# OedonLestrange42/GNURadio-WiFI-ImageTransfer

Measured on NVIDIA B200. Metric: rx_msamples_per_s, higher is better.
Workload: dtype f32+u8

## Files before the change

### gnuradio-wifi-imagetransfer_b200/csrc/rx_kernels.cuh

```cuda
#pragma once
#include <cuda_pipeline.h>
#include "viterbi.cuh"

__device__ __forceinline__ cf fe_at(const cf *x, int64_t j, int hist) { return j < -(int64_t)hist ? cf{0.f, 0.f} : x[j]; }

__device__ __forceinline__ int find_link(const LinkDesc *links, int n_links, int64_t chunk)
{
    int lo = 0, hi = n_links - 1;
    while (lo < hi) {
        int mid = (lo + hi + 1) >> 1;
        if (links[mid].chunk_base <= chunk) lo = mid; else hi = mid - 1;
    }
    return lo;
}

#ifndef DET_BLOCK
#define DET_BLOCK 32
#endif
#define DET_SPLIT (DET_THREADS / DET_BLOCK)
#define DET_ROWS (DET_BLOCK + 2)
#define DET_STRIDE 66
#define DET_SMEM_BYTES (DET_ROWS * DET_STRIDE * (int)sizeof(cf) + 32)

__device__ __forceinline__ uint32_t det_smem_u32(const void *p) { return (uint32_t)__cvta_generic_to_shared(p); }
// ... 472 lines not shown
        if ((tid & 31) == 0) { rmax[tid >> 5] = bm; ridx[tid >> 5] = bi; }
        __syncthreads();
        if (tid == 0) {
            for (int w = 1; w < SL_THREADS / 32; ++w)
                if (rmax[w] > bm || (rmax[w] == bm && ridx[w] < bi)) { bm = rmax[w]; bi = ridx[w]; }
            top[r] = bi;
            smag[bi] = -2.f;
        }
        __syncthreads();
    }
    if (tid == 0) {
        int found = 0, fs = SYNC_LENGTH;
        float fo = 0.f;
        for (int i = 0; i < 3 && found != 64; ++i)
            for (int k = i + 1; k < 4; ++k) {
                int lo = min(top[i], top[k]), hi = max(top[i], top[k]);
                int diff = hi - lo;
                if (diff == 63 || diff == 64 || diff == 65) {
                    cf first = scorr[lo], second = scorr[hi];
                    cf pr = wdm_cmulc(first, second);
                    fs = lo;
                    fo = wdm_atan2f(pr.im, pr.re) / (float)diff;
                    found = diff;
                    if (diff == 64) break;
                }
            }
        frames[f].found = found;
        frames[f].frame_start = fs;
        frames[f].freq_long = fo;
    }
}

#ifndef DEMOD_MINB
#define DEMOD_MINB 5
#endif
struct DemodParams {
    double bw, freq;
    int algo;
    int want_carrier;
    int soft;
};

__device__ __forceinline__ int emitted_symbols(int avail, int fs, bool last)
{
    int R = avail - fs;
    if (R <= 0) return 0;
    int E = R <= 128 ? R : 128 + 64 * ((R - 128) / 80) + max(0, ((R - 128) % 80) - 16);
    return last ? E / 64 : (E + 63) / 64;
}

template <bool SOFT, int ALGO, int PHASE>
__global__ void __launch_bounds__(128, DEMOD_MINB) k_demod(const cf *__restrict__ iq, const LinkDesc *__restrict__ links, wifi_b200_frame *frames, int f0, int n_frames,
                                                EqState *states, uint8_t *rows, cf *carrier, DemodParams prm,
                                                const uint16_t *__restrict__ depunct_lut, uint32_t *__restrict__ vit_in,
                                                int8_t *__restrict__ soft_rows, uint32_t *__restrict__ vit_soft_in)
{
    __shared__ int8_t s_soft[SOFT ? 4 : 1][SOFT ? 392 : 4];
    __shared__ uint16_t s_slut[SOFT ? 4 : 1][SOFT ? 432 : 2];
    __shared__ float s_h2[SOFT ? 4 : 1][SOFT ? 64 : 2];
    __shared__ cf s_hu[4][64];
    __shared__ double s_md[4][64], s_ms[4][64];
    __shared__ uint16_t s_lut[4][432];
    __shared__ __align__(8) uint8_t s_bits[4][49 * 8];
    constexpr int phase = PHASE;
    const int wib = threadIdx.x >> 5, lane = threadIdx.x & 31;
    const int f = f0 + blockIdx.x * 4 + wib;
    if (f >= n_frames) return;
    const wifi_b200_frame F = frames[f];
    if (phase == 1 && F.burst_len < SYNC_LENGTH + 63) return;
    const LinkDesc L = links[F.link];
    const cf *x = iq + L.x_off;
    const bool last = L.is_final && (f == L.frame_first + L.frame_count - 1);
    float fo = F.freq_long;
    if (phase == 0) {
        if (!F.found) {
            fo = L.fo_carry;
            for (int g = f - 1; g >= L.frame_first; --g)
                if (frames[g].found) { fo = frames[g].freq_long; break; }
        }
        if (F.burst_len < SYNC_LENGTH + 63) {
            if (lane == 0 && F.n_syms >= 0) frames[f].freq_long = fo;
            return;
        }
    }
    const int avail = F.burst_len - SYNC_LENGTH;
    const int fs = F.frame_start;
    const int n_syms = emitted_symbols(avail, fs, last);
    const float fshort = F.freq_short;
    const float delta = fo - fshort;
    const cf w1 = crot(delta);
    const int64_t t = F.trigger;
    const int hist = L.hist;

    const int iA = lane + 32, iB = lane;
    const bool usedA = (iA <= 58), usedB = (iB >= 6);
    const bool dcA = (iA == 32);
    const int carA = c_tab.carrier_of[iA], carB = c_tab.carrier_of[iB];
    const float ltsA = c_tab.lts[iA], ltsB = c_tab.lts[iB];
    const int q0 = 2 * dev_bitrev5(lane);
    const WarpTw tw = warp_tw(lane, false);

    cf HA = {0.f, 0.f}, HB = {0.f, 0.f};
    cf pp[4] = {{0.f, 0.f}, {0.f, 0.f}, {0.f, 0.f}, {0.f, 0.f}};
    double d_er = 0.0, eps0, snr = 0.0;
    float havg = 1.f, w0A = 1.f, w0B = 1.f;
    int frame_symbols = 0, enc = 0, nb = 1;
    int n_begin, n_end;
    EqState *st = states + f;
    if (phase == 0) {
        eps0 = ((double)fshort - (double)fo) * prm.bw / (2 * M_PI * prm.freq);
        n_begin = 0;
        n_end = n_syms < 3 ? n_syms : 3;
        if (lane == 0) { frames[f].freq_long = fo; frames[f].n_syms = n_syms; }
    } else {
        if (!F.sig_ok) return;
        frame_symbols = F.frame_symbols;
        enc = F.encoding;
        nb = c_tab.mcs[enc].n_bpsc;
        HA = st->H[iA]; HB = st->H[iB];
#pragma unroll
        for (int q = 0; q < 4; ++q) pp[q] = st->prev_pil[q];
        d_er = st->d_er; eps0 = st->eps0;
        if (SOFT) { havg = st->havg; w0A = st->w0[iA]; w0B = st->w0[iB]; }
        n_begin = 3;
        n_end = n_syms < frame_symbols + 3 ? n_syms : frame_symbols + 3;
    }
    const int ndbps = c_tab.mcs[enc].n_dbps;
    const int wps = (phase == 1 && (ndbps & 7) == 0 && frame_symbols <= WIFI_MAX_SYM && F.length <= WIFI_MAX_PSDU) ? ndbps >> 3 : 0;
    uint32_t era_word = 0;
    if (wps) {
        for (int i = lane; i < 2 * ndbps; i += 32) {
            uint16_t e = depunct_lut[enc * 432 + i];
            s_lut[wib][(i & 15) * 27 + (i >> 4)] = (e == 0xffffu) ? (uint16_t)(48 << 3) : e;
        }
        if (lane < wps)
            for (int k = 0; k < 16; ++k)
                if (depunct_lut[enc * 432 + 16 * lane + k] == 0xffffu) era_word |= 2u << (2 * k);
        if (lane == 0) *reinterpret_cast<uint2 *>(&s_bits[wib][48 * 8]) = make_uint2(0u, 0u);
        __syncwarp();
    }
    uint32_t *vw = vit_in + (int64_t)f * VIT_MAXW;
    const bool soft_on = SOFT && phase == 1;
    const int swps = (soft_on && frame_symbols <= WIFI_MAX_SYM && F.length <= WIFI_MAX_PSDU) ? ndbps >> 1 : 0;
    if (SOFT && soft_on) {
        for (int i = lane; i < 2 * ndbps; i += 32) {
            uint16_t e = depunct_lut[enc * 432 + i];
            s_slut[wib][i] = (e == 0xffffu) ? 384 : e;
        }
        if (lane == 0) s_soft[wib][384] = 0;
        __syncwarp();
    }
    uint32_t *vsw = vit_soft_in ? vit_soft_in + (int64_t)f * SOFT_MAXW : nullptr;
    int n_rows = 0;
    auto sym_j0 = [&](int n) { return fs + ((n < 2) ? 64 * n + q0 : 128 + 80 * (n - 2) + 16 + q0); };
    auto fetch_raw = [&](int n, cf (&raw)[2]) {
        const int j0 = sym_j0(n);
#pragma unroll
        for (int u = 0; u < 2; ++u) {
            const int j = j0 + u;
            const int64_t src = t + j - 16;
            raw[u] = (j < avail && src >= -(int64_t)hist) ? x[src] : cf{0.f, 0.f};
        }
    };
    cf raw[2] = {{0.f, 0.f}, {0.f, 0.f}};
    if (n_begin < n_end) fetch_raw(n_begin, raw);
    int pidx = n_begin >= 2 ? (n_begin - 2) % 127 : 0;
    for (int n = n_begin; n < n_end; ++n) {
        if (PHASE == 1) __builtin_assume(n >= 3);
        cf a, b;
        {
            const int j0 = sym_j0(n);
            const cf s0 = raw[0], s1 = raw[1];
            if (n + 1 < n_end) fetch_raw(n + 1, raw);
            const cf r0 = crot(delta * (float)j0);
            const cf r1 = cmul(r0, w1);
            a = (j0 < avail) ? cmul(s0, r0) : cf{0.f, 0.f};
            b = (j0 + 1 < avail) ? cmul(s1, r1) : cf{0.f, 0.f};
        }
        warp_fft64(a, b, lane, tw);
        {
            double k = 2 * M_PI * n * 80 * (eps0 + d_er);
            double phA = k * (iA - 32) / 64, phB = k * (iB - 32) / 64;
            a = cmul(a, crot((float)phA));
            b = cmul(b, crot((float)phB));
        }
        cf c11 = cshfl(b, 11), c25 = cshfl(b, 25), c39 = cshfl(a, 7), c53 = cshfl(a, 21);
        const float p = (n >= 2) ? c_tab.polarity[pidx] : 1.f;
        if (n >= 2) pidx = pidx == 126 ? 0 : pidx + 1;
        cf pil[4];
        double beta;
        cf sbeta;
        if (n < 2) {
            sbeta = cadd(cadd(csub(c11, c25), c39), c53);
            pil[0] = c11; pil[1] = cf{-c25.re, -c25.im}; pil[2] = c39; pil[3] = c53;
        } else {
            pil[0] = cscale(c11, p); pil[1] = cscale(c25, p); pil[2] = cscale(c39, p); pil[3] = cscale(c53, -p);
            sbeta = cadd(cadd(cadd(pil[0], pil[2]), pil[1]), pil[3]);
        }
        cf ser = {0.f, 0.f};
        if (n >= 2) {
#pragma unroll
            for (int q = 0; q < 4; ++q) ser = wdm_cmacc(ser, pil[q], pp[q]);
        }
        const bool up = lane >= 16;
        const float at = wdm_atan2f(up ? ser.im : sbeta.im, up ? ser.re : sbeta.re);
        beta = (double)__shfl_sync(0xffffffffu, at, 0);
        double er = 0.0;
        if (n >= 2) {
            er = (double)__shfl_sync(0xffffffffu, at, 16);
            er *= prm.bw / (2 * M_PI * prm.freq * 80);
        }
#pragma unroll
        for (int q = 0; q < 4; ++q) pp[q] = pil[q];
        const cf wb = crot((float)(-beta));
        a = cmul(a, wb);
        b = cmul(b, wb);
        if (n >= 2) d_er = (1 - 0.1) * d_er + 0.1 * er;

        if (ALGO == WIFI_EQ_COMB) {
            cf r11 = cmul(c11, wb), r25 = cmul(c25, wb), r39 = cmul(c39, wb), r53 = cmul(c53, wb);
            cf cp[4];
            if (n < 2) { cp[0] = r11; cp[1] = cf{-r25.re, -r25.im}; cp[2] = r39; cp[3] = r53; }
            else { cp[0] = cscale(r11, p); cp[1] = cscale(r25, p); cp[2] = cscale(r39, p); cp[3] = cscale(r53, -p); }
            cf avg = cscale(cadd(cadd(cadd(cp[0], cp[1]), cp[2]), cp[3]), 0.25f);
#pragma unroll
            for (int u = 0; u < 2; ++u) {
                int i = u ? iB : iA;
                cf G;
                if (i <= 11) G = cadd(cscale(avg, (float)(11 - i) / 11.0f), cscale(cp[0], (float)i / 11.0f));
                else if (i <= 25) G = cadd(cscale(cp[0], (float)(25 - i) / 14.0f), cscale(cp[1], (float)(i - 11) / 14.0f));
                else if (i <= 39) G = cadd(cscale(cp[1], (float)(39 - i) / 14.0f), cscale(cp[2], (float)(i - 25) / 14.0f));
                else if (i <= 53) G = cadd(cscale(cp[2], (float)(53 - i) / 14.0f), cscale(cp[3], (float)(i - 39) / 14.0f));
                else G = cadd(cscale(cp[3], (float)(64 - i) / 11.0f), cscale(avg, (float)(i - 53) / 11.0f));
                if (u) b = cdiv(b, G); else a = cdiv(a, G);
            }
        }
        if (n == 0) {
            HA = a; HB = b;
        } else if (n == 1) {
            {
                cf d = csub(HA, a), s = cadd(HA, a);
                float md = sqrtf(d.re * d.re + d.im * d.im), ms = sqrtf(s.re * s.re + s.im * s.im);
                s_md[wib][iA] = (double)md * (double)md; s_ms[wib][iA] = (double)ms * (double)ms;
                if (usedA && !dcA) HA = cdiv(s, cf{ltsA * 2.0f, 0.f});
                d = csub(HB, b); s = cadd(HB, b);
                md = sqrtf(d.re * d.re + d.im * d.im); ms = sqrtf(s.re * s.re + s.im * s.im);
                s_md[wib][iB] = (double)md * (double)md; s_ms[wib][iB] = (double)ms * (double)ms;
                if (usedB) HB = cdiv(s, cf{ltsB * 2.0f, 0.f});
            }
            if (SOFT) {
                s_h2[wib][iA] = HA.re * HA.re + HA.im * HA.im;
                s_h2[wib][iB] = HB.re * HB.re + HB.im * HB.im;
            }
            __syncwarp();
            if (lane == 0) {
                double signal = 0, noise = 0;
                float acc = 0.f;
                for (int i = 6; i <= 58; ++i) {
                    if (i == 32) continue;
                    noise += s_md[wib][i];
                    signal += s_ms[wib][i];
                    if (SOFT) acc += s_h2[wib][i];
                }
                snr = 10 * log10(signal / noise / 2);
                havg = acc / 52.0f;
            }
            if (SOFT) {
                havg = __shfl_sync(0xffffffffu, havg, 0);
                w0A = s_h2[wib][iA] / havg;
                w0B = s_h2[wib][iB] / havg;
            }
            __syncwarp();
        } else {
            cf symA = {0.f, 0.f}, symB = {0.f, 0.f};
            int bitsA = 0, bitsB = 0;
            cf huA = {0.f, 0.f}, huB = {0.f, 0.f};
            SoftQ sqA, sqB;
#pragma unroll
            for (int u = 0; u < 2; ++u)
#pragma unroll
                for (int t = 0; t < 3; ++t) { sqA.q[u][t] = 0; sqB.q[u][t] = 0; }
            if (carA >= 0) {
                cf ptA;
                symA = cdiv(a, HA);
                dev_decide_point(nb, symA, bitsA, ptA);
                if (SOFT && soft_on) sqA = dev_soft_demap(nb, symA, w0A);
                if (ALGO == WIFI_EQ_LMS) {
                    cf q = cdiv(a, ptA);
                    HA = cadd(cscale(HA, 0.5f), cscale(q, 0.5f));
                } else if (ALGO == WIFI_EQ_STA) huA = cdiv(a, ptA);
            } else if (iA == 39) huA = cscale(a, p);
            else if (iA == 53) huA = cscale(a, -p);
            if (carB >= 0) {
                cf ptB;
                symB = cdiv(b, HB);
                dev_decide_point(nb, symB, bitsB, ptB);
                if (SOFT && soft_on) sqB = dev_soft_demap(nb, symB, w0B);
                if (ALGO == WIFI_EQ_LMS) {
                    cf q = cdiv(b, ptB);
                    HB = cadd(cscale(HB, 0.5f), cscale(q, 0.5f));
                } else if (ALGO == WIFI_EQ_STA) huB = cdiv(b, ptB);
            } else if (iB == 11 || iB == 25) huB = cscale(b, p);
            if (ALGO == WIFI_EQ_STA) {
                s_hu[wib][iA] = huA; s_hu[wib][iB] = huB;
                __syncwarp();
#pragma unroll
                for (int u = 0; u < 2; ++u) {
                    int i = u ? iB : iA;
                    if (i < 6 || i > 58 || i == 32) continue;
                    cf sum = {0.f, 0.f};
                    int cnt = 0;
                    for (int k = i - 2; k <= i + 2; ++k) {
                        if (k == 32 || k < 6 || k > 58) continue;
                        sum = cadd(sum, s_hu[wib][k]);
                        ++cnt;
                    }
                    cf avg = {sum.re / (float)cnt, sum.im / (float)cnt};
                    if (u) HB = cadd(cscale(HB, 0.5f), cscale(avg, 0.5f));
                    else HA = cadd(cscale(HA, 0.5f), cscale(avg, 0.5f));
                }
                __syncwarp();
            }
            if (n == 2) {
                if (carA >= 0) st->sig_bits[carA] = (uint8_t)bitsA;
                if (carB >= 0) st->sig_bits[carB] = (uint8_t)bitsB;
            } else {
                int64_t row = F.row_off + (n - 3);
                if (carA >= 0) rows[row * 48 + carA] = (uint8_t)bitsA;
                if (carB >= 0) rows[row * 48 + carB] = (uint8_t)bitsB;
                if (prm.want_carrier) {
                    if (carA >= 0) carrier[row * 48 + carA] = symA;
                    if (carB >= 0) carrier[row * 48 + carB] = symB;
                }
                if (wps) {
                    if (carA >= 0)
                        *reinterpret_cast<uint2 *>(&s_bits[wib][carA * 8]) =
                            make_uint2((((uint32_t)bitsA & 15u) * 0x00204081u) & 0x01010101u, (((uint32_t)bitsA >> 4) * 0x81u) & 0x0101u);
                    if (carB >= 0)
                        *reinterpret_cast<uint2 *>(&s_bits[wib][carB * 8]) =
                            make_uint2((((uint32_t)bitsB & 15u) * 0x00204081u) & 0x01010101u, (((uint32_t)bitsB >> 4) * 0x81u) & 0x0101u);
                    __syncwarp();
                    if (lane < wps) {
                        uint32_t word = era_word;
#pragma unroll
                        for (int k = 0; k < 16; ++k) {
                            const uint32_t e = s_lut[wib][k * 27 + lane];
                            word += (uint32_t)s_bits[wib][e] << (2 * k);
                        }
                        vw[(n - 3) * wps + lane] = word;
                    }
                    __syncwarp();
                }
                if (SOFT && soft_on) {
                    const int hb = nb > 1 ? nb >> 1 : 1;
#pragma unroll
                    for (int u = 0; u < 2; ++u)
#pragma unroll
                        for (int t = 0; t < 3; ++t) {
                            if (t < hb && (u == 0 || nb > 1)) {
                                const int k = u * hb + t;
                                if (carA >= 0) { s_soft[wib][(carA << 3) | k] = (int8_t)sqA.q[u][t]; soft_rows[row * SOFT_ROW + carA * nb + k] = (int8_t)sqA.q[u][t]; }
                                if (carB >= 0) { s_soft[wib][(carB << 3) | k] = (int8_t)sqB.q[u][t]; soft_rows[row * SOFT_ROW + carB * nb + k] = (int8_t)sqB.q[u][t]; }
                            }
                        }
                    __syncwarp();
                    for (int w = lane; w < swps; w += 32) {
                        uint32_t word = 0;
#pragma unroll
                        for (int k = 0; k < 4; ++k) word |= (uint32_t)(uint8_t)s_soft[wib][s_slut[wib][4 * w + k]] << (8 * k);
                        vsw[(n - 3) * swps + w] = word;
                    }
                    __syncwarp();
                }
                ++n_rows;
            }
        }
    }
    if (phase == 0) {
        st->H[iA] = HA; st->H[iB] = HB;
        if (SOFT) { st->w0[iA] = w0A; st->w0[iB] = w0B; }
        if (lane == 0) {
#pragma unroll
            for (int q = 0; q < 4; ++q) st->prev_pil[q] = pp[q];
            st->d_er = d_er; st->eps0 = eps0; st->snr = snr; st->havg = havg;
        }
    } else if (lane == 0) {
        frames[f].n_rows = n_rows;
    }
}

__global__ void __launch_bounds__(VIT_BLOCK) k_signal(wifi_b200_frame *frames, int f0, int n_frames, const EqState *states)
{
    __shared__ uint32_t ring[5 * 16 * VIT_BLOCK];
    __shared__ uint4 s_bm[8 * 4 * 16];
    const int tid = threadIdx.x;
    for (int i = tid; i < 512; i += VIT_BLOCK) s_bm[i] = VitCoreH::table_entry(i >> 6, (i >> 4) & 3, (uint32_t)(i & 15));
    __syncthreads();
    int f = f0 + blockIdx.x * VIT_BLOCK + tid;
    if (f >= n_frames) return;
    if (frames[f].n_syms < 3) return;
    const EqState *st = states + f;
    uint64_t lo = 0, hi = 0;
    for (int tstep = 0; tstep < 24; ++tstep) {
        int i0 = 2 * tstep, i1 = i0 + 1;
        uint32_t s0 = st->sig_bits[(i0 % 16) * 3 + i0 / 16] & 1u, s1 = st->sig_bits[(i1 % 16) * 3 + i1 / 16] & 1u;
        uint64_t nib = s0 | (s1 << 2);
        if (tstep < 16) lo |= nib << (4 * tstep); else hi |= nib << (4 * (tstep - 16));
    }
    VitCoreH v;
    v.init();
    const uint32_t first = (uint32_t)lo;
    v.step4<0>(s_bm, 0xau, 0xau, first & 0xfu, (first >> 4) & 0xfu);
    v.step4<4>(s_bm, (first >> 8) & 0xfu, (first >> 12) & 0xfu, (first >> 16) & 0xfu, (first >> 20) & 0xfu);
    v.trace_begin(ring, 1, 5, tid, true, 0xfcu);
    uint32_t dec = 0;
#pragma unroll 1
    for (int chunk = 1; chunk < 8; ++chunk) {
        const uint32_t bits = (uint32_t)(lo >> 24);
        lo = (lo >> 32) | (hi << 32);
// ... 499 lines not shown
```

### gnuradio-wifi-imagetransfer_b200/csrc/wifi_b200.cu

```cuda
#include <sched.h>

#include <cfloat>
#include <cmath>
#include <cstdio>
#include <cstdlib>
#include <cstring>
#include <mutex>
#include <string>
#include <deque>
#include <vector>

#include "rx_kernels.cuh"
#include "tx_kernels.cuh"


namespace {

const McsDesc H_MCS[8] = {
    {1, 48, 24, 0x0D, 0}, {1, 48, 36, 0x0F, 2}, {2, 96, 48, 0x05, 0}, {2, 96, 72, 0x07, 2},
    {4, 192, 96, 0x09, 0}, {4, 192, 144, 0x0B, 2}, {6, 288, 192, 0x01, 1}, {6, 288, 216, 0x03, 2},
};
const int H_LTS53[53] = {1, 1, -1, -1, 1, 1, -1, 1, -1, 1, 1, 1, 1, 1, 1, -1, -1, 1, 1, -1, 1, -1, 1, 1, 1, 1, 0,
                         1, -1, -1, 1, 1, -1, 1, -1, 1, -1, -1, -1, -1, -1, 1, 1, -1, -1, 1, -1, 1, -1, 1, 1, 1, 1};

// ... 490 lines not shown
        }
        if (timed) mark(h, ST_DETECT);
        if (tiles_g > 0)
            k_detect<<<(unsigned)(DET_SPLIT * tiles_g), DET_BLOCK, DET_SMEM, s>>>(iq, gl, ng, tile_base, tile_base + tiles_g, thr_f, h->d_flags, h->d_summary);
        if (timed) mark(h, ST_SELECT);
        if (tiles_g > 0)
            k_select_spec<<<(unsigned)((tiles_g * 32 + 127) / 128), 128, 0, s>>>(h->d_flags, h->d_summary, gl, ng, tile_base, tile_base + tiles_g,
                                                                                h->cfg.min_plateau, h->d_spec_trig, h->d_spec_cnt);
        if (tiles_g > 0)
            k_select_fix<<<(unsigned)((tiles_g * 32 + 127) / 128), 128, 0, s>>>(h->d_flags, h->d_summary, gl, ng, tile_base, tile_base + tiles_g,
                                                                               h->cfg.min_plateau, h->d_spec_trig, h->d_spec_cnt, h->d_spec_trig2, h->d_spec_cnt2);
        k_select<<<(ng * 32 + 127) / 128, 128, 0, s>>>(h->d_flags, h->d_summary, gl, ng, h->cfg.min_plateau, h->d_trig_tmp, h->d_spec_trig, h->d_spec_cnt2,
                                                       h->d_spec_trig2);
        k_reserve<<<1, 1024, 0, s>>>(gl, ng, h->d_counters, (unsigned long long *)(h->d_counters + 8), h->cfg.max_frames, h->d_counters + 2,
                                     (long long)frame_base, (long long)row_base);
        k_frames_init<<<dim3(8, ng), 128, 0, s>>>(gl, h->d_trig_tmp, h->d_frames, lb);
        if (timed) mark(h, ST_SYNC_LONG);
        CK(cudaMemcpyAsync(h->h_counters, h->d_counters, 64, cudaMemcpyDeviceToHost, s));
        CK(cudaStreamSynchronize(s));
        if (h->h_counters[2] != 0 || h->h_counters[0] > h->cfg.max_frames) {
            h->err = "more sync_short triggers than max_frames";
            return WIFI_E_OVERFLOW;
        }
        const int64_t f_end = h->h_counters[0], nf = f_end - frame_base;
        const int64_t rows_needed = *(int64_t *)(h->h_counters + 8);
        if (rows_needed > h->row_cap) {
            h->err = "row capacity exceeded";
            return WIFI_E_OVERFLOW;
        }
        const int f0 = (int)frame_base, fe = (int)f_end;
        if (nf > 0) {
            k_sync_long<<<(unsigned)nf, SL_THREADS, 0, s>>>(iq, h->d_links, h->d_frames, f0, fe);
            if (timed) mark(h, ST_DEMOD_HEAD);
            demod_head<<<(unsigned)((nf + 3) / 4), 128, 0, s>>>(iq, h->d_links, h->d_frames, f0, fe, h->d_states, h->d_rows, h->d_carrier, prm,
                                                            h->d_depunct, h->d_vit_in, h->d_soft, h->d_vit_soft_in);
            if (timed) mark(h, ST_SIGNAL);
            k_signal<<<(unsigned)((nf + VIT_BLOCK - 1) / VIT_BLOCK), VIT_BLOCK, 0, s>>>(h->d_frames, f0, fe, h->d_states);
            if (timed) mark(h, ST_DEMOD_DATA);
            demod_data<<<(unsigned)((nf + 3) / 4), 128, 0, s>>>(iq, h->d_links, h->d_frames, f0, fe, h->d_states, h->d_rows, h->d_carrier, prm,
                                                            h->d_depunct, h->d_vit_in, h->d_soft, h->d_vit_soft_in);
            if (timed) mark(h, ST_PLAN);
            CK(cudaMemsetAsync(h->d_link_dirty + lb, 0, (size_t)ng * sizeof(int), s));
            CK(cudaMemsetAsync(h->d_link_dirty + MAX_LINKS + lb, 0xff, (size_t)ng * sizeof(int), s));
            CK(cudaMemsetAsync(h->d_counters + 1, 0, sizeof(int), s));
            k_plan_fast<<<(unsigned)((nf + 127) / 128), 128, 0, s>>>(h->d_frames, f0, fe, h->d_jobs, h->d_pack_list, h->d_counters + 1, h->d_link_dirty, soft);
            k_plan<<<(ng * 32 + 127) / 128, 128, 0, s>>>(gl, ng, h->d_frames, h->d_jobs, h->d_pack_list, h->d_counters + 1,
                                                         h->d_counters + 2, soft, h->d_link_dirty + lb, h->d_link_dirty + MAX_LINKS + lb);
            if (timed) mark(h, ST_PACK);
            if (!soft) {
                k_pack<<<dim3(7, 148), 256, 0, s>>>(h->d_jobs, h->d_pack_list, h->d_counters + 1, h->d_rows, h->d_depunct, h->d_vit_in, h->d_frames);
                if (timed) mark(h, ST_VITERBI);
                auto launch_viterbi = [&](cudaStream_t st, int a, int b) {
                    const int64_t n = b - a;
                    const int form = h->viterbi_form ? h->viterbi_form : (n <= VW_SWITCH ? 1 : (n <= VQ_SWITCH ? 2 : 3));
                    if (form == 1) k_viterbi_warp<<<(unsigned)((n + VW_WARPS - 1) / VW_WARPS), 32 * VW_WARPS, 0, st>>>(h->d_jobs, a, b, h->d_vit_in, h->d_psdu, h->d_frames);
                    else if (form == 2) k_viterbi_quad<<<(unsigned)((n + VQ_FRAMES - 1) / VQ_FRAMES), VQ_BLOCK, 0, st>>>(h->d_jobs, a, b, h->d_vit_in, h->d_psdu, h->d_frames);
                    else k_viterbi<<<(unsigned)((n + VIT_BLOCK - 1) / VIT_BLOCK), VIT_BLOCK, vit_smem, st>>>(h->d_jobs, a, b, h->d_vit_in, h->d_psdu, h->d_frames);
                };
                const int64_t wave = (int64_t)h->sm_count * 2 * VIT_BLOCK;
                int64_t rem = nf % wave;
                if (rem > VQ_SPLIT_MAX) rem = 0;
                if (h->viterbi_form || nf < wave || rem == 0) {
                    launch_viterbi(s, f0, fe);
                } else {
                    CK(cudaEventRecord(h->ev_fork, s));
                    CK(cudaStreamWaitEvent(h->aux_stream, h->ev_fork, 0));
                    launch_viterbi(h->aux_stream, fe - (int)rem, fe);
                    launch_viterbi(s, f0, fe - (int)rem);
                    CK(cudaEventRecord(h->ev_join, h->aux_stream));
                    CK(cudaStreamWaitEvent(s, h->ev_join, 0));
                }
            } else {
// ... 1125 lines not shown
```

### gnuradio-wifi-imagetransfer_b200/csrc/wifi_common.cuh

```cuda
#pragma once
#include <cuda_runtime.h>
#include <stdint.h>
#include "../../include/wifi_b200.h"
#include "../../include/wifi_detmath.h"

#define WIFI_MAX_SYM 511
#define WIFI_MAX_PSDU 1528
#define SS_MIN_GAP 480
#define SS_MAX_SAMPLES 43200
#define SYNC_LENGTH 320
#define FE_CHUNK 64
#define DET_THREADS 128
#define DET_TILE (DET_THREADS * FE_CHUNK)
#define PSDU_STRIDE 1536
#define VIT_MAXW 1560
#define SOFT_MAXW 6240
#define SOFT_ROW 288

typedef wdm_cf cf;
__device__ __forceinline__ cf cadd(cf a, cf b) { return {a.re + b.re, a.im + b.im}; }
__device__ __forceinline__ cf csub(cf a, cf b) { return {a.re - b.re, a.im - b.im}; }
__device__ __forceinline__ cf cmul(cf a, cf b) { return wdm_cmul(a, b); }
__device__ __forceinline__ cf cdiv(cf a, cf b) { return wdm_cdiv(a, b); }
__device__ __forceinline__ cf cscale(cf a, float s) { return {a.re * s, a.im * s}; }
// ... 131 lines not shown
#pragma unroll
    for (int s = 0; s < 5; ++s) {
        const int half = 1 << s;
        t.w[s] = c_tab.tw[(lane & (half - 1)) * (32 >> s)];
    }
    t.w[5] = c_tab.tw[lane];
    if (inverse) {
#pragma unroll
        for (int s = 0; s < 6; ++s) t.w[s].im = -t.w[s].im;
    }
    return t;
}

__device__ __forceinline__ void warp_fft64(cf &a, cf &b, int lane, const WarpTw &tw)
{
#pragma unroll
    for (int s = 0; s < 5; ++s) {
        const int half = 1 << s;
        const cf w = tw.w[s];
        const bool hi = (lane & half) != 0;
        cf ta = hi ? cmul(w, a) : a;
        cf tb = hi ? cmul(w, b) : b;
        cf ra = cshfl_xor(ta, half);
        cf rb = cshfl_xor(tb, half);
        a = hi ? csub(ra, ta) : cadd(a, ra);
        b = hi ? csub(rb, tb) : cadd(b, rb);
    }
    cf t = cmul(tw.w[5], b);
    cf u = a;
    a = cadd(u, t);
    b = csub(u, t);
}

__device__ __forceinline__ int dev_soft_q(float l, float w)
{
    float v = rintf((l * w) * 16.0f);
    if (v > 32.f) v = 32.f;
    if (v < -32.f) v = -32.f;
    if (!(v == v)) v = 0.f;
    return (int)v;
}
struct SoftQ { int q[2][3]; };
__device__ __forceinline__ SoftQ dev_soft_demap(int nb, cf s, float w)
{
    SoftQ r;
#pragma unroll
    for (int u = 0; u < 2; ++u)
#pragma unroll
        for (int t = 0; t < 3; ++t) r.q[u][t] = 0;
    if (nb == 1) { r.q[0][0] = dev_soft_q(s.re, w); return r; }
    const int h = nb >> 1;
    const float level = (h == 1) ? sqrtf(0.5f) : (h == 2) ? sqrtf(0.1f) : sqrtf(1.0f / 42.0f);
    const float ax[2] = {s.re / level, s.im / level};
#pragma unroll
    for (int u = 0; u < 2; ++u) {
        const float a = ax[u], m = fabsf(a);
        r.q[u][0] = dev_soft_q(a, w);
        if (h == 2) r.q[u][1] = dev_soft_q(2.0f - m, w);
        if (h == 3) {
            r.q[u][1] = dev_soft_q(4.0f - m, w);
            r.q[u][2] = dev_soft_q(2.0f - fabsf(m - 4.0f), w);
        }
    }
    return r;
}
```

Before: 46750.

## Process each frame with a half-warp in demod, eight frames per block

The demod kernel now maps one frame to 16 lanes instead of a full warp. Each lane holds four FFT bins and uses a new half-warp radix FFT (four shuffle stages plus two in-register stages). Depuncture words are built from a uint4-vectorised LUT, and launch bounds and the grid are retuned to eight frames per block. The aim is to cut shuffle count and idle lanes per frame and raise frame-level parallelism. The cost is more registers, predicated execution to keep half-warps in lockstep, and extra loop iterations when the two frames sharing a warp differ in symbol count.

After: 49500, median of 6. 5.9% higher.

```diff
diff --git a/gnuradio-wifi-imagetransfer_b200/csrc/rx_kernels.cuh b/gnuradio-wifi-imagetransfer_b200/csrc/rx_kernels.cuh
--- a/gnuradio-wifi-imagetransfer_b200/csrc/rx_kernels.cuh
+++ b/gnuradio-wifi-imagetransfer_b200/csrc/rx_kernels.cuh
@@ -528,8 +528,9 @@
 }
 
 #ifndef DEMOD_MINB
-#define DEMOD_MINB 5
+#define DEMOD_MINB 4
 #endif
+#define DEMOD_FPB 8
 struct DemodParams {
     double bw, freq;
     int algo;
@@ -546,37 +547,40 @@
 }
 
 template <bool SOFT, int ALGO, int PHASE>
-__global__ void __launch_bounds__(128, DEMOD_MINB) k_demod(const cf *__restrict__ iq, const LinkDesc *__restrict__ links, wifi_b200_frame *frames, int f0, int n_frames,
+__global__ void __launch_bounds__(32 * DEMOD_FPB / 2, DEMOD_MINB) k_demod(const cf *__restrict__ iq, const LinkDesc *__restrict__ links, wifi_b200_frame *frames, int f0, int n_frames,
                                                 EqState *states, uint8_t *rows, cf *carrier, DemodParams prm,
                                                 const uint16_t *__restrict__ depunct_lut, uint32_t *__restrict__ vit_in,
                                                 int8_t *__restrict__ soft_rows, uint32_t *__restrict__ vit_soft_in)
 {
-    __shared__ int8_t s_soft[SOFT ? 4 : 1][SOFT ? 392 : 4];
-    __shared__ uint16_t s_slut[SOFT ? 4 : 1][SOFT ? 432 : 2];
-    __shared__ float s_h2[SOFT ? 4 : 1][SOFT ? 64 : 2];
-    __shared__ cf s_hu[4][64];
-    __shared__ double s_md[4][64], s_ms[4][64];
-    __shared__ uint16_t s_lut[4][432];
-    __shared__ __align__(8) uint8_t s_bits[4][49 * 8];
+    constexpr int BITS = 49 * 8;
+    __shared__ int8_t s_soft[SOFT ? DEMOD_FPB * BITS : 4];
+    __shared__ uint16_t s_slut[SOFT ? DEMOD_FPB : 1][SOFT ? 432 : 2];
+    __shared__ float s_h2[SOFT ? DEMOD_FPB : 1][SOFT ? 64 : 2];
+    __shared__ cf s_hu[DEMOD_FPB][64];
+    __shared__ double s_md[DEMOD_FPB][64], s_ms[DEMOD_FPB][64];
+    __shared__ __align__(16) uint32_t s_lut[DEMOD_FPB][27 * 20];
+    __shared__ __align__(8) uint8_t s_bits[DEMOD_FPB * BITS];
     constexpr int phase = PHASE;
-    const int wib = threadIdx.x >> 5, lane = threadIdx.x & 31;
-    const int f = f0 + blockIdx.x * 4 + wib;
-    if (f >= n_frames) return;
-    const wifi_b200_frame F = frames[f];
-    if (phase == 1 && F.burst_len < SYNC_LENGTH + 63) return;
+    const int fib = threadIdx.x >> 4, l = threadIdx.x & 15;
+    const unsigned hmask = 0xffffu << (threadIdx.x & 16);
+    const int f = f0 + blockIdx.x * DEMOD_FPB + fib;
+    if (f0 + blockIdx.x * DEMOD_FPB + (fib & ~1) >= n_frames) return;
+    bool ok = f < n_frames;
+    const wifi_b200_frame F = frames[ok ? f : f - 1];
+    if (phase == 1 && F.burst_len < SYNC_LENGTH + 63) ok = false;
     const LinkDesc L = links[F.link];
     const cf *x = iq + L.x_off;
     const bool last = L.is_final && (f == L.frame_first + L.frame_count - 1);
     float fo = F.freq_long;
-    if (phase == 0) {
+    if (phase == 0 && ok) {
         if (!F.found) {
             fo = L.fo_carry;
             for (int g = f - 1; g >= L.frame_first; --g)
                 if (frames[g].found) { fo = frames[g].freq_long; break; }
         }
         if (F.burst_len < SYNC_LENGTH + 63) {
-            if (lane == 0 && F.n_syms >= 0) frames[f].freq_long = fo;
-            return;
+            if (l == 0 && F.n_syms >= 0) frames[f].freq_long = fo;
+            ok = false;
         }
     }
     const int avail = F.burst_len - SYNC_LENGTH;
@@ -588,99 +592,117 @@
     const int64_t t = F.trigger;
     const int hist = L.hist;
 
-    const int iA = lane + 32, iB = lane;
-    const bool usedA = (iA <= 58), usedB = (iB >= 6);
-    const bool dcA = (iA == 32);
-    const int carA = c_tab.carrier_of[iA], carB = c_tab.carrier_of[iB];
-    const float ltsA = c_tab.lts[iA], ltsB = c_tab.lts[iB];
-    const int q0 = 2 * dev_bitrev5(lane);
-    const WarpTw tw = warp_tw(lane, false);
-
-    cf HA = {0.f, 0.f}, HB = {0.f, 0.f};
+    int bin[4], car[4];
+#pragma unroll
+    for (int k = 0; k < 4; ++k) {
+        bin[k] = (l + 16 * k + 32) & 63;
+        car[k] = c_tab.carrier_of[bin[k]];
+    }
+    const int q0 = 4 * (int)(__brev((unsigned)l) >> 28);
+    const HalfTw tw = half_tw(l);
+
+    cf H[4] = {{0.f, 0.f}, {0.f, 0.f}, {0.f, 0.f}, {0.f, 0.f}};
+    float w0[4] = {1.f, 1.f, 1.f, 1.f};
     cf pp[4] = {{0.f, 0.f}, {0.f, 0.f}, {0.f, 0.f}, {0.f, 0.f}};
     double d_er = 0.0, eps0, snr = 0.0;
-    float havg = 1.f, w0A = 1.f, w0B = 1.f;
+    float havg = 1.f;
     int frame_symbols = 0, enc = 0, nb = 1;
     int n_begin, n_end;
     EqState *st = states + f;
     if (phase == 0) {
         eps0 = ((double)fshort - (double)fo) * prm.bw / (2 * M_PI * prm.freq);
         n_begin = 0;
-        n_end = n_syms < 3 ? n_syms : 3;
-        if (lane == 0) { frames[f].freq_long = fo; frames[f].n_syms = n_syms; }
+        n_end = !ok ? 0 : n_syms < 3 ? n_syms : 3;
+        if (ok && l == 0) { frames[f].freq_long = fo; frames[f].n_syms = n_syms; }
     } else {
-        if (!F.sig_ok) return;
+        ok = ok && F.sig_ok;
+        n_begin = n_end = 3;
+    }
+    if (phase == 1 && ok) {
         frame_symbols = F.frame_symbols;
         enc = F.encoding;
         nb = c_tab.mcs[enc].n_bpsc;
-        HA = st->H[iA]; HB = st->H[iB];
+#pragma unroll
+        for (int k = 0; k < 4; ++k) H[k] = st->H[bin[k]];
 #pragma unroll
         for (int q = 0; q < 4; ++q) pp[q] = st->prev_pil[q];
         d_er = st->d_er; eps0 = st->eps0;
-        if (SOFT) { havg = st->havg; w0A = st->w0[iA]; w0B = st->w0[iB]; }
-        n_begin = 3;
+        if (SOFT) {
+            havg = st->havg;
+#pragma unroll
+            for (int k = 0; k < 4; ++k) w0[k] = st->w0[bin[k]];
+        }
         n_end = n_syms < frame_symbols + 3 ? n_syms : frame_symbols + 3;
     }
     const int ndbps = c_tab.mcs[enc].n_dbps;
-    const int wps = (phase == 1 && (ndbps & 7) == 0 && frame_symbols <= WIFI_MAX_SYM && F.length <= WIFI_MAX_PSDU) ? ndbps >> 3 : 0;
-    uint32_t era_word = 0;
+    const int wps = (phase == 1 && ok && (ndbps & 7) == 0 && frame_symbols <= WIFI_MAX_SYM && F.length <= WIFI_MAX_PSDU) ? ndbps >> 3 : 0;
+    uint32_t era_word[2] = {0u, 0u};
     if (wps) {
-        for (int i = lane; i < 2 * ndbps; i += 32) {
-            uint16_t e = depunct_lut[enc * 432 + i];
-            s_lut[wib][(i & 15) * 27 + (i >> 4)] = (e == 0xffffu) ? (uint16_t)(48 << 3) : e;
-        }
-        if (lane < wps)
-            for (int k = 0; k < 16; ++k)
-                if (depunct_lut[enc * 432 + 16 * lane + k] == 0xffffu) era_word |= 2u << (2 * k);
-        if (lane == 0) *reinterpret_cast<uint2 *>(&s_bits[wib][48 * 8]) = make_uint2(0u, 0u);
-        __syncwarp();
+        for (int i = l; i < 2 * ndbps; i += 16) {
+            const uint16_t e = depunct_lut[enc * 432 + i];
+            s_lut[fib][(i >> 4) * 20 + (i & 15)] = fib * BITS + ((e == 0xffffu) ? 48 << 3 : e);
+        }
+#pragma unroll
+        for (int j = 0; j < 2; ++j) {
+            const int w = l + 16 * j;
+            if (w < wps)
+                for (int k = 0; k < 16; ++k)
+                    if (depunct_lut[enc * 432 + 16 * w + k] == 0xffffu) era_word[j] |= 2u << (2 * k);
+        }
+        if (l == 0) *reinterpret_cast<uint2 *>(&s_bits[fib * BITS + 48 * 8]) = make_uint2(0u, 0u);
+        __syncwarp(hmask);
     }
     uint32_t *vw = vit_in + (int64_t)f * VIT_MAXW;
     const bool soft_on = SOFT && phase == 1;
-    const int swps = (soft_on && frame_symbols <= WIFI_MAX_SYM && F.length <= WIFI_MAX_PSDU) ? ndbps >> 1 : 0;
-    if (SOFT && soft_on) {
-        for (int i = lane; i < 2 * ndbps; i += 32) {
-            uint16_t e = depunct_lut[enc * 432 + i];
-            s_slut[wib][i] = (e == 0xffffu) ? 384 : e;
-        }
-        if (lane == 0) s_soft[wib][384] = 0;
-        __syncwarp();
+    const int swps = (soft_on && ok && frame_symbols <= WIFI_MAX_SYM && F.length <= WIFI_MAX_PSDU) ? ndbps >> 1 : 0;
+    if (SOFT && swps) {
+        for (int i = l; i < 2 * ndbps; i += 16) {
+            const uint16_t e = depunct_lut[enc * 432 + i];
+            s_slut[fib][i] = (uint16_t)(fib * BITS + ((e == 0xffffu) ? 384 : e));
+        }
+        if (l == 0) s_soft[fib * BITS + 384] = 0;
+        __syncwarp(hmask);
     }
     uint32_t *vsw = vit_soft_in ? vit_soft_in + (int64_t)f * SOFT_MAXW : nullptr;
     int n_rows = 0;
     auto sym_j0 = [&](int n) { return fs + ((n < 2) ? 64 * n + q0 : 128 + 80 * (n - 2) + 16 + q0); };
-    auto fetch_raw = [&](int n, cf (&raw)[2]) {
+    auto fetch_raw = [&](int n, cf (&raw)[4]) {
         const int j0 = sym_j0(n);
 #pragma unroll
-        for (int u = 0; u < 2; ++u) {
+        for (int u = 0; u < 4; ++u) {
             const int j = j0 + u;
             const int64_t src = t + j - 16;
             raw[u] = (j < avail && src >= -(int64_t)hist) ? x[src] : cf{0.f, 0.f};
         }
     };
-    cf raw[2] = {{0.f, 0.f}, {0.f, 0.f}};
+    cf raw[4] = {{0.f, 0.f}, {0.f, 0.f}, {0.f, 0.f}, {0.f, 0.f}};
     if (n_begin < n_end) fetch_raw(n_begin, raw);
     int pidx = n_begin >= 2 ? (n_begin - 2) % 127 : 0;
-    for (int n = n_begin; n < n_end; ++n) {
+    const int n_stop = max(n_end, __shfl_xor_sync(0xffffffffu, n_end, 16));
+    for (int n = n_begin; n < n_stop; ++n) {
         if (PHASE == 1) __builtin_assume(n >= 3);
-        cf a, b;
+        const bool act = n < n_end;
+        cf v[4];
         {
             const int j0 = sym_j0(n);
-            const cf s0 = raw[0], s1 = raw[1];
+            const cf s0 = raw[0], s1 = raw[1], s2 = raw[2], s3 = raw[3];
             if (n + 1 < n_end) fetch_raw(n + 1, raw);
             const cf r0 = crot(delta * (float)j0);
             const cf r1 = cmul(r0, w1);
-            a = (j0 < avail) ? cmul(s0, r0) : cf{0.f, 0.f};
-            b = (j0 + 1 < avail) ? cmul(s1, r1) : cf{0.f, 0.f};
-        }
-        warp_fft64(a, b, lane, tw);
+            const cf r2 = crot(delta * (float)(j0 + 2));
+            const cf r3 = cmul(r2, w1);
+            v[0] = (j0 < avail) ? cmul(s0, r0) : cf{0.f, 0.f};
+            v[2] = (j0 + 1 < avail) ? cmul(s1, r1) : cf{0.f, 0.f};
+            v[1] = (j0 + 2 < avail) ? cmul(s2, r2) : cf{0.f, 0.f};
+            v[3] = (j0 + 3 < avail) ? cmul(s3, r3) : cf{0.f, 0.f};
+        }
+        half_fft64(v, l, tw);
         {
-            double k = 2 * M_PI * n * 80 * (eps0 + d_er);
-            double phA = k * (iA - 32) / 64, phB = k * (iB - 32) / 64;
-            a = cmul(a, crot((float)phA));
-            b = cmul(b, crot((float)phB));
-        }
-        cf c11 = cshfl(b, 11), c25 = cshfl(b, 25), c39 = cshfl(a, 7), c53 = cshfl(a, 21);
+            const double k = 2 * M_PI * n * 80 * (eps0 + d_er);
+#pragma unroll
+            for (int u = 0; u < 4; ++u) v[u] = cmul(v[u], crot((float)(k * (bin[u] - 32) / 64)));
+        }
+        cf c11 = cshfl16(v[2], 11), c25 = cshfl16(v[3], 9), c39 = cshfl16(v[0], 7), c53 = cshfl16(v[1], 5);
         const float p = (n >= 2) ? c_tab.polarity[pidx] : 1.f;
         if (n >= 2) pidx = pidx == 126 ? 0 : pidx + 1;
         cf pil[4];
@@ -698,20 +720,22 @@
 #pragma unroll
             for (int q = 0; q < 4; ++q) ser = wdm_cmacc(ser, pil[q], pp[q]);
         }
-        const bool up = lane >= 16;
+        const bool up = l >= 8;
         const float at = wdm_atan2f(up ? ser.im : sbeta.im, up ? ser.re : sbeta.re);
-        beta = (double)__shfl_sync(0xffffffffu, at, 0);
+        beta = (double)__shfl_sync(0xffffffffu, at, 0, 16);
         double er = 0.0;
         if (n >= 2) {
-            er = (double)__shfl_sync(0xffffffffu, at, 16);
+            er = (double)__shfl_sync(0xffffffffu, at, 8, 16);
             er *= prm.bw / (2 * M_PI * prm.freq * 80);
         }
-#pragma unroll
-        for (int q = 0; q < 4; ++q) pp[q] = pil[q];
+        if (act) {
+#pragma unroll
+            for (int q = 0; q < 4; ++q) pp[q] = pil[q];
+        }
         const cf wb = crot((float)(-beta));
-        a = cmul(a, wb);
-        b = cmul(b, wb);
-        if (n >= 2) d_er = (1 - 0.1) * d_er + 0.1 * er;
+#pragma unroll
+        for (int u = 0; u < 4; ++u) v[u] = cmul(v[u], wb);
+        if (n >= 2 && act) d_er = (1 - 0.1) * d_er + 0.1 * er;
 
         if (ALGO == WIFI_EQ_COMB) {
             cf r11 = cmul(c11, wb), r25 = cmul(c25, wb), r39 = cmul(c39, wb), r53 = cmul(c53, wb);
@@ -720,167 +744,171 @@
             else { cp[0] = cscale(r11, p); cp[1] = cscale(r25, p); cp[2] = cscale(r39, p); cp[3] = cscale(r53, -p); }
             cf avg = cscale(cadd(cadd(cadd(cp[0], cp[1]), cp[2]), cp[3]), 0.25f);
 #pragma unroll
-            for (int u = 0; u < 2; ++u) {
-                int i = u ? iB : iA;
+            for (int u = 0; u < 4; ++u) {
+                const int i = bin[u];
                 cf G;
                 if (i <= 11) G = cadd(cscale(avg, (float)(11 - i) / 11.0f), cscale(cp[0], (float)i / 11.0f));
                 else if (i <= 25) G = cadd(cscale(cp[0], (float)(25 - i) / 14.0f), cscale(cp[1], (float)(i - 11) / 14.0f));
                 else if (i <= 39) G = cadd(cscale(cp[1], (float)(39 - i) / 14.0f), cscale(cp[2], (float)(i - 25) / 14.0f));
                 else if (i <= 53) G = cadd(cscale(cp[2], (float)(53 - i) / 14.0f), cscale(cp[3], (float)(i - 39) / 14.0f));
                 else G = cadd(cscale(cp[3], (float)(64 - i) / 11.0f), cscale(avg, (float)(i - 53) / 11.0f));
-                if (u) b = cdiv(b, G); else a = cdiv(a, G);
+                v[u] = cdiv(v[u], G);
             }
         }
         if (n == 0) {
-            HA = a; HB = b;
+            if (act) {
+#pragma unroll
+                for (int u = 0; u < 4; ++u) H[u] = v[u];
+            }
         } else if (n == 1) {
-            {
-                cf d = csub(HA, a), s = cadd(HA, a);
-                float md = sqrtf(d.re * d.re + d.im * d.im), ms = sqrtf(s.re * s.re + s.im * s.im);
-                s_md[wib][iA] = (double)md * (double)md; s_ms[wib][iA] = (double)ms * (double)ms;
-                if (usedA && !dcA) HA = cdiv(s, cf{ltsA * 2.0f, 0.f});
-                d = csub(HB, b); s = cadd(HB, b);
-                md = sqrtf(d.re * d.re + d.im * d.im); ms = sqrtf(s.re * s.re + s.im * s.im);
-                s_md[wib][iB] = (double)md * (double)md; s_ms[wib][iB] = (double)ms * (double)ms;
-                if (usedB) HB = cdiv(s, cf{ltsB * 2.0f, 0.f});
-            }
-            if (SOFT) {
-                s_h2[wib][iA] = HA.re * HA.re + HA.im * HA.im;
-                s_h2[wib][iB] = HB.re * HB.re + HB.im * HB.im;
-            }
-            __syncwarp();
-            if (lane == 0) {
+#pragma unroll
+            for (int u = 0; u < 4; ++u) {
+                const int i = bin[u];
+                const cf d = csub(H[u], v[u]), s = cadd(H[u], v[u]);
+                const float md = sqrtf(d.re * d.re + d.im * d.im), ms = sqrtf(s.re * s.re + s.im * s.im);
+                s_md[fib][i] = (double)md * (double)md; s_ms[fib][i] = (double)ms * (double)ms;
+                if (act && i >= 6 && i <= 58 && i != 32) H[u] = cdiv(s, cf{c_tab.lts[i] * 2.0f, 0.f});
+                if (SOFT) s_h2[fib][i] = H[u].re * H[u].re + H[u].im * H[u].im;
+            }
+            __syncwarp(hmask);
+            if (act && l == 0) {
                 double signal = 0, noise = 0;
                 float acc = 0.f;
                 for (int i = 6; i <= 58; ++i) {
                     if (i == 32) continue;
-                    noise += s_md[wib][i];
-                    signal += s_ms[wib][i];
-                    if (SOFT) acc += s_h2[wib][i];
+                    noise += s_md[fib][i];
+                    signal += s_ms[fib][i];
+                    if (SOFT) acc += s_h2[fib][i];
                 }
                 snr = 10 * log10(signal / noise / 2);
                 havg = acc / 52.0f;
             }
             if (SOFT) {
-                havg = __shfl_sync(0xffffffffu, havg, 0);
-                w0A = s_h2[wib][iA] / havg;
-                w0B = s_h2[wib][iB] / havg;
-            }
-            __syncwarp();
+                havg = __shfl_sync(0xffffffffu, havg, 0, 16);
+                if (act) {
+#pragma unroll
+                    for (int u = 0; u < 4; ++u) w0[u] = s_h2[fib][bin[u]] / havg;
+                }
+            }
+            __syncwarp(hmask);
         } else {
-            cf symA = {0.f, 0.f}, symB = {0.f, 0.f};
-            int bitsA = 0, bitsB = 0;
-            cf huA = {0.f, 0.f}, huB = {0.f, 0.f};
-            SoftQ sqA, sqB;
-#pragma unroll
-            for (int u = 0; u < 2; ++u)
-#pragma unroll
-                for (int t = 0; t < 3; ++t) { sqA.q[u][t] = 0; sqB.q[u][t] = 0; }
-            if (carA >= 0) {
-                cf ptA;
-                symA = cdiv(a, HA);
-                dev_decide_point(nb, symA, bitsA, ptA);
-                if (SOFT && soft_on) sqA = dev_soft_demap(nb, symA, w0A);
-                if (ALGO == WIFI_EQ_LMS) {
-                    cf q = cdiv(a, ptA);
-                    HA = cadd(cscale(HA, 0.5f), cscale(q, 0.5f));
-                } else if (ALGO == WIFI_EQ_STA) huA = cdiv(a, ptA);
-            } else if (iA == 39) huA = cscale(a, p);
-            else if (iA == 53) huA = cscale(a, -p);
-            if (carB >= 0) {
-                cf ptB;
-                symB = cdiv(b, HB);
-                dev_decide_point(nb, symB, bitsB, ptB);
-                if (SOFT && soft_on) sqB = dev_soft_demap(nb, symB, w0B);
-                if (ALGO == WIFI_EQ_LMS) {
-                    cf q = cdiv(b, ptB);
-                    HB = cadd(cscale(HB, 0.5f), cscale(q, 0.5f));
-                } else if (ALGO == WIFI_EQ_STA) huB = cdiv(b, ptB);
-            } else if (iB == 11 || iB == 25) huB = cscale(b, p);
+            cf sym[4], hu[4];
+            int bits[4];
+            const int64_t row = F.row_off + (n - 3);
+#pragma unroll
+            for (int u = 0; u < 4; ++u) {
+                const int i = bin[u];
+                sym[u] = hu[u] = cf{0.f, 0.f};
+                bits[u] = 0;
+                if (act && car[u] >= 0) {
+                    cf pt;
+                    sym[u] = cdiv(v[u], H[u]);
+                    dev_decide_point(nb, sym[u], bits[u], pt);
+                    if (SOFT && soft_on) {
+                        const SoftQ sq = dev_soft_demap(nb, sym[u], w0[u]);
+                        const int hb = nb > 1 ? nb >> 1 : 1;
+#pragma unroll
+                        for (int a = 0; a < 2; ++a)
+#pragma unroll
+                            for (int b = 0; b < 3; ++b) {
+                                if (b < hb && (a == 0 || nb > 1)) {
+                                    const int k = a * hb + b;
+                                    s_soft[fib * BITS + ((car[u] << 3) | k)] = (int8_t)sq.q[a][b];
+                                    soft_rows[row * SOFT_ROW + car[u] * nb + k] = (int8_t)sq.q[a][b];
+                                }
+                            }
+                    }
+                    if (ALGO == WIFI_EQ_LMS) {
+                        const cf q = cdiv(v[u], pt);
+                        H[u] = cadd(cscale(H[u], 0.5f), cscale(q, 0.5f));
+                    } else if (ALGO == WIFI_EQ_STA) hu[u] = cdiv(v[u], pt);
+                } else if (i == 11 || i == 25 || i == 39) hu[u] = cscale(v[u], p);
+                else if (i == 53) hu[u] = cscale(v[u], -p);
+            }
             if (ALGO == WIFI_EQ_STA) {
-                s_hu[wib][iA] = huA; s_hu[wib][iB] = huB;
-                __syncwarp();
-#pragma unroll
-                for (int u = 0; u < 2; ++u) {
-                    int i = u ? iB : iA;
-                    if (i < 6 || i > 58 || i == 32) continue;
+#pragma unroll
+                for (int u = 0; u < 4; ++u) s_hu[fib][bin[u]] = hu[u];
+                __syncwarp(hmask);
+#pragma unroll
+                for (int u = 0; u < 4; ++u) {
+                    const int i = bin[u];
+                    if (!act || i < 6 || i > 58 || i == 32) continue;
                     cf sum = {0.f, 0.f};
                     int cnt = 0;
                     for (int k = i - 2; k <= i + 2; ++k) {
                         if (k == 32 || k < 6 || k > 58) continue;
-                        sum = cadd(sum, s_hu[wib][k]);
+                        sum = cadd(sum, s_hu[fib][k]);
                         ++cnt;
                     }
                     cf avg = {sum.re / (float)cnt, sum.im / (float)cnt};
-                    if (u) HB = cadd(cscale(HB, 0.5f), cscale(avg, 0.5f));
-                    else HA = cadd(cscale(HA, 0.5f), cscale(avg, 0.5f));
+                    H[u] = cadd(cscale(H[u], 0.5f), cscale(avg, 0.5f));
                 }
-                __syncwarp();
+                __syncwarp(hmask);
             }
             if (n == 2) {
-                if (carA >= 0) st->sig_bits[carA] = (uint8_t)bitsA;
-                if (carB >= 0) st->sig_bits[carB] = (uint8_t)bitsB;
+#pragma unroll
+                for (int u = 0; u < 4; ++u)
+                    if (act && car[u] >= 0) st->sig_bits[car[u]] = (uint8_t)bits[u];
             } else {
-                int64_t row = F.row_off + (n - 3);
-                if (carA >= 0) rows[row * 48 + carA] = (uint8_t)bitsA;
-                if (carB >= 0) rows[row * 48 + carB] = (uint8_t)bitsB;
-                if (prm.want_carrier) {
-                    if (carA >= 0) carrier[row * 48 + carA] = symA;
-                    if (carB >= 0) carrier[row * 48 + carB] = symB;
+#pragma unroll
+                for (int u = 0; u < 4; ++u)
+                    if (act && car[u] >= 0) {
+                        rows[row * 48 + car[u]] = (uint8_t)bits[u];
+                        if (prm.want_carrier) carrier[row * 48 + car[u]] = sym[u];
+                    }
+                if (wps && act) {
+#pragma unroll
+                    for (int u = 0; u < 4; ++u)
+                        if (car[u] >= 0)
+                            *reinterpret_cast<uint2 *>(&s_bits[fib * BITS + car[u] * 8]) =
+                                make_uint2((((uint32_t)bits[u] & 15u) * 0x00204081u) & 0x01010101u, (((uint32_t)bits[u] >> 4) * 0x81u) & 0x0101u);
+                    __syncwarp(hmask);
+#pragma unroll
+                    for (int j = 0; j < 2; ++j) {
+                        const int w = l + 16 * j;
+                        if (w < wps) {
+                            uint32_t word = era_word[j];
+                            const uint4 *e4 = reinterpret_cast<const uint4 *>(&s_lut[fib][w * 20]);
+#pragma unroll
+                            for (int q = 0; q < 4; ++q) {
+                                const uint4 e = e4[q];
+                                word += (uint32_t)s_bits[e.x] << (8 * q);
+                                word += (uint32_t)s_bits[e.y] << (8 * q + 2);
+                                word += (uint32_t)s_bits[e.z] << (8 * q + 4);
+                                word += (uint32_t)s_bits[e.w] << (8 * q + 6);
+                            }
+                            vw[(n - 3) * wps + w] = word;
+                        }
+                    }
+                    __syncwarp(hmask);
                 }
-                if (wps) {
-                    if (carA >= 0)
-                        *reinterpret_cast<uint2 *>(&s_bits[wib][carA * 8]) =
-                            make_uint2((((uint32_t)bitsA & 15u) * 0x00204081u) & 0x01010101u, (((uint32_t)bitsA >> 4) * 0x81u) & 0x0101u);
-                    if (carB >= 0)
-                        *reinterpret_cast<uint2 *>(&s_bits[wib][carB * 8]) =
-                            make_uint2((((uint32_t)bitsB & 15u) * 0x00204081u) & 0x01010101u, (((uint32_t)bitsB >> 4) * 0x81u) & 0x0101u);
-                    __syncwarp();
-                    if (lane < wps) {
-                        uint32_t word = era_word;
-#pragma unroll
-                        for (int k = 0; k < 16; ++k) {
-                            const uint32_t e = s_lut[wib][k * 27 + lane];
-                            word += (uint32_t)s_bits[wib][e] << (2 * k);
-                        }
-                        vw[(n - 3) * wps + lane] = word;
-                    }
-                    __syncwarp();
-                }
-                if (SOFT && soft_on) {
-                    const int hb = nb > 1 ? nb >> 1 : 1;
-#pragma unroll
-                    for (int u = 0; u < 2; ++u)
-#pragma unroll
-                        for (int t = 0; t < 3; ++t) {
-                            if (t < hb && (u == 0 || nb > 1)) {
-                                const int k = u * hb + t;
-                                if (carA >= 0) { s_soft[wib][(carA << 3) | k] = (int8_t)sqA.q[u][t]; soft_rows[row * SOFT_ROW + carA * nb + k] = (int8_t)sqA.q[u][t]; }
-                                if (carB >= 0) { s_soft[wib][(carB << 3) | k] = (int8_t)sqB.q[u][t]; soft_rows[row * SOFT_ROW + carB * nb + k] = (int8_t)sqB.q[u][t]; }
-                            }
-                        }
-                    __syncwarp();
-                    for (int w = lane; w < swps; w += 32) {
+                if (SOFT && swps && act) {
+                    __syncwarp(hmask);
+                    for (int w = l; w < swps; w += 16) {
                         uint32_t word = 0;
 #pragma unroll
-                        for (int k = 0; k < 4; ++k) word |= (uint32_t)(uint8_t)s_soft[wib][s_slut[wib][4 * w + k]] << (8 * k);
+                        for (int k = 0; k < 4; ++k) word |= (uint32_t)(uint8_t)s_soft[s_slut[fib][4 * w + k]] << (8 * k);
                         vsw[(n - 3) * swps + w] = word;
                     }
-                    __syncwarp();
+                    __syncwarp(hmask);
                 }
-                ++n_rows;
-            }
-        }
-    }
+                n_rows += act;
+            }
+        }
+    }
+    if (!ok) return;
     if (phase == 0) {
-        st->H[iA] = HA; st->H[iB] = HB;
-        if (SOFT) { st->w0[iA] = w0A; st->w0[iB] = w0B; }
-        if (lane == 0) {
+#pragma unroll
+        for (int u = 0; u < 4; ++u) {
+            st->H[bin[u]] = H[u];
+            if (SOFT) st->w0[bin[u]] = w0[u];
+        }
+        if (l == 0) {
 #pragma unroll
             for (int q = 0; q < 4; ++q) st->prev_pil[q] = pp[q];
             st->d_er = d_er; st->eps0 = eps0; st->snr = snr; st->havg = havg;
         }
-    } else if (lane == 0) {
+    } else if (l == 0) {
         frames[f].n_rows = n_rows;
     }
 }
diff --git a/gnuradio-wifi-imagetransfer_b200/csrc/wifi_b200.cu b/gnuradio-wifi-imagetransfer_b200/csrc/wifi_b200.cu
--- a/gnuradio-wifi-imagetransfer_b200/csrc/wifi_b200.cu
+++ b/gnuradio-wifi-imagetransfer_b200/csrc/wifi_b200.cu
@@ -546,12 +546,12 @@
         if (nf > 0) {
             k_sync_long<<<(unsigned)nf, SL_THREADS, 0, s>>>(iq, h->d_links, h->d_frames, f0, fe);
             if (timed) mark(h, ST_DEMOD_HEAD);
-            demod_head<<<(unsigned)((nf + 3) / 4), 128, 0, s>>>(iq, h->d_links, h->d_frames, f0, fe, h->d_states, h->d_rows, h->d_carrier, prm,
+            demod_head<<<(unsigned)((nf + DEMOD_FPB - 1) / DEMOD_FPB), 32 * DEMOD_FPB / 2, 0, s>>>(iq, h->d_links, h->d_frames, f0, fe, h->d_states, h->d_rows, h->d_carrier, prm,
                                                             h->d_depunct, h->d_vit_in, h->d_soft, h->d_vit_soft_in);
             if (timed) mark(h, ST_SIGNAL);
             k_signal<<<(unsigned)((nf + VIT_BLOCK - 1) / VIT_BLOCK), VIT_BLOCK, 0, s>>>(h->d_frames, f0, fe, h->d_states);
             if (timed) mark(h, ST_DEMOD_DATA);
-            demod_data<<<(unsigned)((nf + 3) / 4), 128, 0, s>>>(iq, h->d_links, h->d_frames, f0, fe, h->d_states, h->d_rows, h->d_carrier, prm,
+            demod_data<<<(unsigned)((nf + DEMOD_FPB - 1) / DEMOD_FPB), 32 * DEMOD_FPB / 2, 0, s>>>(iq, h->d_links, h->d_frames, f0, fe, h->d_states, h->d_rows, h->d_carrier, prm,
                                                             h->d_depunct, h->d_vit_in, h->d_soft, h->d_vit_soft_in);
             if (timed) mark(h, ST_PLAN);
             CK(cudaMemsetAsync(h->d_link_dirty + lb, 0, (size_t)ng * sizeof(int), s));
diff --git a/gnuradio-wifi-imagetransfer_b200/csrc/wifi_common.cuh b/gnuradio-wifi-imagetransfer_b200/csrc/wifi_common.cuh
--- a/gnuradio-wifi-imagetransfer_b200/csrc/wifi_common.cuh
+++ b/gnuradio-wifi-imagetransfer_b200/csrc/wifi_common.cuh
@@ -187,6 +187,53 @@
     b = csub(u, t);
 }
 
+__device__ __forceinline__ cf cshfl16(cf v, int src) { return {__shfl_sync(0xffffffffu, v.re, src, 16), __shfl_sync(0xffffffffu, v.im, src, 16)}; }
+
+struct HalfTw { cf w[7]; };
+__device__ __forceinline__ HalfTw half_tw(int l)
+{
+    HalfTw t;
+#pragma unroll
+    for (int s = 0; s < 4; ++s) {
+        const int half = 1 << s;
+        t.w[s] = c_tab.tw[(l & (half - 1)) * (32 >> s)];
+    }
+    t.w[4] = c_tab.tw[2 * l];
+    t.w[5] = c_tab.tw[l];
+    t.w[6] = c_tab.tw[l + 16];
+    return t;
+}
+
+__device__ __forceinline__ void half_fft64(cf (&x)[4], int l, const HalfTw &tw)
+{
+#pragma unroll
+    for (int s = 0; s < 4; ++s) {
+        const int half = 1 << s;
+        const cf w = tw.w[s];
+        const bool hi = (l & half) != 0;
+#pragma unroll
+        for (int k = 0; k < 4; ++k) {
+            const cf t = hi ? cmul(w, x[k]) : x[k];
+            const cf r = cshfl_xor(t, half);
+            x[k] = hi ? csub(r, t) : cadd(x[k], r);
+        }
+    }
+#pragma unroll
+    for (int k = 0; k < 4; k += 2) {
+        const cf t = cmul(tw.w[4], x[k + 1]);
+        const cf u = x[k];
+        x[k] = cadd(u, t);
+        x[k + 1] = csub(u, t);
+    }
+#pragma unroll
+    for (int k = 0; k < 2; ++k) {
+        const cf t = cmul(tw.w[5 + k], x[k + 2]);
+        const cf u = x[k];
+        x[k] = cadd(u, t);
+        x[k + 2] = csub(u, t);
+    }
+}
+
 __device__ __forceinline__ int dev_soft_q(float l, float w)
 {
     float v = rintf((l * w) * 16.0f);
```
